# jihun1998/AO

Measured on AMD Instinct MI355X. Metric: points/sec fwd+bwd PTv2m2 S3DIS, higher is better.
Workload: dtype fp32

## Files before the change

### ao_amd/csrc/gemm.hip

```cpp
#include <algorithm>

#include "common.h"

namespace gemm {

constexpr int BM = 64;
constexpr int THREADS = 256;
template <int KC>
__device__ __forceinline__ int lds_slot(int row, int k4) {
    return row * (KC + 8) + 4 * (k4 ^ (row & (KC == 32 ? 1 : 3)));
}

typedef float v4f __attribute__((ext_vector_type(4)));

struct GemmMulti {
    const float *X[3], *W[3], *bias[3];
    float *Y[3];
    int count;
    int sum;
    const float *xsc, *xsh;
    float *stats[3];
    const float *bnx, *bnm, *bnr, *bng, *bnb;
    int bnrelu;
    float *brec;
};

template <int CTRL>
__device__ __forceinline__ float dpp_mov(float v) {
    return __int_as_float(__builtin_amdgcn_update_dpp(0, __float_as_int(v), CTRL, 0xF, 0xF, true));
}
__device__ __forceinline__ float row16_sum(float v) {
    v += dpp_mov<0xB1>(v);
    v += dpp_mov<0x4E>(v);
    v += dpp_mov<0x141>(v);
    v += dpp_mov<0x140>(v);
    return v;
}

template <int BN>
// ... 11 lines not shown
        float4 v = make_float4(acc[t][0], acc[t][1], acc[t][2], acc[t][3]);
        {
            const float4 bb = ptv2_ld_or_zero((const float4 *)(bias + col), bias && col < n);
            v.x += bb.x; v.y += bb.y; v.z += bb.z; v.w += bb.w;
        }
        val[t] = v;
        if (row < m && col < n) {
            float4 *dst = (float4 *)(Y + row * n + col);
            if (accumulate) {
                const float4 o = *dst;
                v.x += o.x; v.y += o.y; v.z += o.z; v.w += o.w;
            }
            *dst = v;
        }
    }
    if (multi.count && multi.brec) {
        float *sS = sX;
        const bool rv = row < m;
        const int cl = (lane >> 4) * 4;
        __syncthreads();
#pragma unroll
        for (int t = 0; t < NT; ++t) {
            const int col = n0 + t * 16 + cl;
            float4 d = make_float4(0.f, 0.f, 0.f, 0.f), e = d;
            if (rv && col < n) {
                const float4 xv = *(const float4 *)(multi.bnx + row * n + col);
                const float4 mm = *(const float4 *)(multi.bnm + col), rs = *(const float4 *)(multi.bnr + col);
                float4 h;
                h.x = (xv.x - mm.x) * rs.x; h.y = (xv.y - mm.y) * rs.y; h.z = (xv.z - mm.z) * rs.z; h.w = (xv.w - mm.w) * rs.w;
                d = val[t];
                if (multi.bnrelu) {
                    const float4 gg = *(const float4 *)(multi.bng + col), bb = *(const float4 *)(multi.bnb + col);
                    if (__builtin_fmaf(h.x, gg.x, bb.x) <= 0.f) d.x = 0.f;
                    if (__builtin_fmaf(h.y, gg.y, bb.y) <= 0.f) d.y = 0.f;
                    if (__builtin_fmaf(h.z, gg.z, bb.z) <= 0.f) d.z = 0.f;
                    if (__builtin_fmaf(h.w, gg.w, bb.w) <= 0.f) d.w = 0.f;
                }
                e = make_float4(d.x * h.x, d.y * h.y, d.z * h.z, d.w * h.w);
            }
            const float ax = row16_sum(d.x), ay = row16_sum(d.y), az = row16_sum(d.z), aw = row16_sum(d.w);
            const float bx = row16_sum(e.x), by = row16_sum(e.y), bz = row16_sum(e.z), bw = row16_sum(e.w);
            if ((lane & 15) == 0) {
                *(float4 *)(sS + (wid * 2 + 0) * BN + t * 16 + cl) = make_float4(ax, ay, az, aw);
                *(float4 *)(sS + (wid * 2 + 1) * BN + t * 16 + cl) = make_float4(bx, by, bz, bw);
            }
        }
        __syncthreads();
        for (int e = tid; e < 2 * BN; e += THREADS) {
            const int which = e / BN, cc = e - which * BN;
            if (n0 + cc < n) {
                float a = sS[which * BN + cc];
#pragma unroll
                for (int w = 1; w < 4; ++w) a += sS[(w * 2 + which) * BN + cc];
                multi.brec[(size_t)rb * 2 * n + (size_t)which * n + n0 + cc] = a;
            }
        }
    }
    float *stats = multi.count ? multi.stats[indep ? z : 0] : nullptr;
    if (stats) {
        float *sS = sX;
        const bool rv = row < m;
        const int cnt = (int)((m - row0) < BM ? (m - row0) : BM);
        const int cl = (lane >> 4) * 4;
        __syncthreads();
#pragma unroll
        for (int t = 0; t < NT; ++t) {
            const float sx = row16_sum(rv ? val[t].x : 0.f), sy = row16_sum(rv ? val[t].y : 0.f);
            const float sz = row16_sum(rv ? val[t].z : 0.f), sw = row16_sum(rv ? val[t].w : 0.f);
            if ((lane & 15) == 0) *(float4 *)(sS + wid * BN + t * 16 + cl) = make_float4(sx, sy, sz, sw);
// ... 29 lines not shown
                if (col < n) {
                    float4 a = *(const float4 *)(sS + t * 16 + cl);
#pragma unroll
                    for (int w = 1; w < 4; ++w) {
                        const float4 o = *(const float4 *)(sS + w * BN + t * 16 + cl);
                        a.x += o.x; a.y += o.y; a.z += o.z; a.w += o.w;
                    }
                    *(float4 *)(stats + (size_t)rb * 2 * n + n + col) = a;
                }
            }
        }
    }
}

template <int BN, bool W_KMAJOR, int KC, bool BF16>
__global__ __launch_bounds__(THREADS) void rows_gemm_kernel(int m, int n, int k, const float *__restrict__ X0,
                                                            const float *__restrict__ W0,
                                                            const float *__restrict__ bias0, float *__restrict__ Y0,
                                                            int accumulate, int ncb, GemmMulti multi) {
    constexpr int PITCH = KC + 8;
    __shared__ __attribute__((aligned(16))) float sX[BM * PITCH];
    __shared__ __attribute__((aligned(16))) float sW[BN * PITCH];
    constexpr int NT = BN / 16;
    constexpr int KQ = KC / 4;
    constexpr int XLOADS = BM * KQ / THREADS;
    constexpr int WQ = BN * KQ;
    constexpr int WLOADS = (WQ + THREADS - 1) / THREADS;
    constexpr int RUN = KC / 16;
    const int tid = threadIdx.x, lane = tid & 63, wid = tid >> 6;
    const int rb = blockIdx.x / ncb, cb = blockIdx.x - rb * ncb;
    const long long row0 = (long long)rb * BM;
    const int n0 = cb * BN;
    const int z = blockIdx.y;
    const bool indep = multi.count && !multi.sum;
    const float *bias = indep ? multi.bias[z] : bias0;
    float *Y = multi.count ? multi.Y[indep ? z : 0] : Y0;
    const int npair = (multi.count && multi.sum) ? multi.count : 1;
    const float *X = multi.count ? multi.X[indep ? z : 0] : X0;
    const float *W = multi.count ? multi.W[indep ? z : 0] : W0;

    float4 rx[XLOADS], rw[WLOADS];
    auto fetch = [&](int k0) {
#pragma unroll
        for (int j = 0; j < XLOADS; ++j) {
            const int q = tid + j * THREADS, r = q / KQ, kq = (q % KQ) * 4;
            const long long row = row0 + r;
            rx[j] = ptv2_ld_or_zero((const float4 *)(X + row * k + k0 + kq), row < m && k0 + kq < k);
            if (multi.xsc && k0 + kq < k) {
                const float4 s4 = *(const float4 *)(multi.xsc + k0 + kq), h4 = *(const float4 *)(multi.xsh + k0 + kq);
                rx[j].x = fmaxf(__builtin_fmaf(rx[j].x, s4.x, h4.x), 0.f);
                rx[j].y = fmaxf(__builtin_fmaf(rx[j].y, s4.y, h4.y), 0.f);
                rx[j].z = fmaxf(__builtin_fmaf(rx[j].z, s4.z, h4.z), 0.f);
                rx[j].w = fmaxf(__builtin_fmaf(rx[j].w, s4.w, h4.w), 0.f);
            }
        }
#pragma unroll
        for (int j = 0; j < WLOADS; ++j) {
            const int q = tid + j * THREADS;
            {
                if (!W_KMAJOR) {
                    const int r = q / KQ, kq = (q % KQ) * 4;
                    rw[j] = ptv2_ld_or_zero((const float4 *)(W + (long long)(n0 + r) * k + k0 + kq), q < WQ && n0 + r < n && k0 + kq < k);
                } else {
                    const int kk = q % KC, cq = (q / KC) * 4;
// ... 71 lines not shown
                        acc[t] = __builtin_amdgcn_mfma_f32_16x16x4f32(w4.x, xr[j].x, acc[t], 0, 0, 0);
                        acc[t] = __builtin_amdgcn_mfma_f32_16x16x4f32(w4.y, xr[j].y, acc[t], 0, 0, 0);
                        acc[t] = __builtin_amdgcn_mfma_f32_16x16x4f32(w4.z, xr[j].z, acc[t], 0, 0, 0);
                        acc[t] = __builtin_amdgcn_mfma_f32_16x16x4f32(w4.w, xr[j].w, acc[t], 0, 0, 0);
                    }
                }
            }
            if (more) {
                __syncthreads();
                stash();
                __syncthreads();
            }
        }
    }
    gemm_epilogue<BN>(acc, row0, rb, n0, z, indep, m, n, bias, Y, accumulate, multi, sX);
}

template <int BN, bool W_KMAJOR, int K, bool BF16>
__global__ __launch_bounds__(THREADS) void rows_gemm_direct_kernel(int m, int n, const float *__restrict__ X0,
                                                                   const float *__restrict__ W0, const float *__restrict__ bias0,
                                                                   float *__restrict__ Y0, int accumulate, int ncb, GemmMulti multi) {
    constexpr int NT = BN / 16, QF = K / 16, LDW = K + 8, KQ = K / 4;
    extern __shared__ float4 gd_lds4[];
    float *sW = (float *)gd_lds4;
    float *sSc = sW + (size_t)BN * LDW;
    const int tid = threadIdx.x, lane = tid & 63, wid = tid >> 6, l15 = lane & 15, q = lane >> 4;
    const int rb = blockIdx.x / ncb, cb = blockIdx.x - rb * ncb;
    const long long row0 = (long long)rb * BM;
    const int n0 = cb * BN;
    const int z = blockIdx.y;
    const bool indep = multi.count && !multi.sum;
    const float *bias = indep ? multi.bias[z] : bias0;
    float *Y = multi.count ? multi.Y[indep ? z : 0] : Y0;
    const int npair = (multi.count && multi.sum) ? multi.count : 1;
    const float *X = multi.count ? multi.X[indep ? z : 0] : X0;
    const float *W = multi.count ? multi.W[indep ? z : 0] : W0;
    const long long row = row0 + wid * 16 + l15;
    const bool rv = row < m;

    v4f acc[NT];
#pragma unroll
    for (int t = 0; t < NT; ++t) acc[t] = (v4f){0.f, 0.f, 0.f, 0.f};
    if (multi.xsc)
        for (int e = tid; e < K; e += THREADS) { sSc[e] = multi.xsc[e]; sSc[K + e] = multi.xsh[e]; }
    for (int pair = 0; pair < npair; ++pair) {
        if (pair > 0) {
            X = multi.X[pair];
            W = multi.W[pair];
            __syncthreads();
        }
        float4 x[QF];
        const float *xr = rv ? X + row * K + 4 * q : ptv2_zero_pad;
#pragma unroll
        for (int j = 0; j < QF; ++j) x[j] = *(const float4 *)(xr + 16 * j);
        if (!W_KMAJOR) {
            constexpr int WL = (BN * KQ + THREADS - 1) / THREADS;
#pragma unroll
            for (int b0 = 0; b0 < WL; b0 += 8) {
                float4 w4[8];
// ... 27 lines not shown
                }
#pragma unroll
                for (int i = 0; i < 8; ++i) {
                    if (b0 + i < WL) {
                        const int e = tid + (b0 + i) * THREADS;
                        const int kk = e % K, cq = (e / K) * 4;
                        if (e < (BN / 4) * K) {
                            sW[(size_t)(cq + 0) * LDW + kk] = w4[i].x; sW[(size_t)(cq + 1) * LDW + kk] = w4[i].y;
                            sW[(size_t)(cq + 2) * LDW + kk] = w4[i].z; sW[(size_t)(cq + 3) * LDW + kk] = w4[i].w;
                        }
                    }
                }
            }
        }
        __syncthreads();
        if (multi.xsc) {
#pragma unroll
            for (int j = 0; j < QF; ++j) {
                const float4 s4 = *(const float4 *)(sSc + 16 * j + 4 * q), h4 = *(const float4 *)(sSc + K + 16 * j + 4 * q);
                x[j].x = fmaxf(__builtin_fmaf(x[j].x, s4.x, h4.x), 0.f); x[j].y = fmaxf(__builtin_fmaf(x[j].y, s4.y, h4.y), 0.f);
                x[j].z = fmaxf(__builtin_fmaf(x[j].z, s4.z, h4.z), 0.f); x[j].w = fmaxf(__builtin_fmaf(x[j].w, s4.w, h4.w), 0.f);
            }
        }
        const float *pw = sW + (size_t)l15 * LDW + 4 * q;
        if constexpr (BF16) {
#pragma unroll
            for (int j = 0; j < QF; j += 2) {
                const float4 x1 = j + 1 < QF ? x[j + 1] : make_float4(0.f, 0.f, 0.f, 0.f);
                const ptv2_bf16x8 xb = ptv2_pack_bf16(x[j], x1);
#pragma unroll
                for (int t = 0; t < NT; ++t) {
// ... 26 lines not shown
                                                                   int ncb, GemmMulti multi) {
    constexpr int NT = BN / 16, QF = K / 16, JW = (QF + 3) / 4;
    __shared__ __attribute__((aligned(16))) float sRed[4][NT][64 * 4];
    const int tid = threadIdx.x, lane = tid & 63, wid = tid >> 6, l15 = lane & 15, q = lane >> 4;
    const int rb = blockIdx.x / ncb, cb = blockIdx.x - rb * ncb;
    const long long row0 = (long long)rb * 16;
    const int n0 = cb * BN;
    const int z = blockIdx.y;
    const bool indep = multi.count && !multi.sum;
    const float *bias = indep ? multi.bias[z] : bias0;
    float *Y = multi.count ? multi.Y[indep ? z : 0] : Y0;
    const int npair = (multi.count && multi.sum) ? multi.count : 1;
    const long long row = row0 + l15;
    const bool rv = row < m;
    const int j0 = wid * JW;
    v4f acc[NT];
#pragma unroll
    for (int t = 0; t < NT; ++t) acc[t] = (v4f){0.f, 0.f, 0.f, 0.f};
    for (int pair = 0; pair < npair; ++pair) {
        const float *X = multi.count ? multi.X[indep ? z : pair] : X0;
        const float *W = multi.count ? multi.W[indep ? z : pair] : W0;
        float4 x[JW], w[JW][NT], s4[JW], h4[JW];
        const float *xr = rv ? X + row * K + 4 * q : ptv2_zero_pad;
#pragma unroll
        for (int jj = 0; jj < JW; ++jj) {
            const int j = j0 + jj;
            const bool jok = j < QF;
            x[jj] = *(const float4 *)((jok && rv) ? xr + 16 * j : ptv2_zero_pad);
            if (multi.xsc) {
                s4[jj] = *(const float4 *)(jok ? multi.xsc + 16 * j + 4 * q : ptv2_zero_pad);
                h4[jj] = *(const float4 *)(jok ? multi.xsh + 16 * j + 4 * q : ptv2_zero_pad);
            }
#pragma unroll
            for (int t = 0; t < NT; ++t) {
                const int col = n0 + 16 * t + l15;
                const bool ok = jok && col < n;
                if (!W_KMAJOR) {
                    w[jj][t] = *(const float4 *)(ok ? W + (long long)col * K + 16 * j + 4 * q : ptv2_zero_pad);
                } else {
                    const float *wp = ok ? W + (long long)(16 * j + 4 * q) * n + col : ptv2_zero_pad;
                    const long long st = ok ? n : 0;
                    w[jj][t] = make_float4(wp[0], wp[st], wp[2 * st], wp[3 * st]);
                }
            }
        }
#pragma unroll
        for (int jj = 0; jj < JW; ++jj) {
            if (multi.xsc) {
                x[jj].x = fmaxf(__builtin_fmaf(x[jj].x, s4[jj].x, h4[jj].x), 0.f); x[jj].y = fmaxf(__builtin_fmaf(x[jj].y, s4[jj].y, h4[jj].y), 0.f);
                x[jj].z = fmaxf(__builtin_fmaf(x[jj].z, s4[jj].z, h4[jj].z), 0.f); x[jj].w = fmaxf(__builtin_fmaf(x[jj].w, s4[jj].w, h4[jj].w), 0.f);
                if (!rv) x[jj] = make_float4(0.f, 0.f, 0.f, 0.f);
            }
#pragma unroll
            for (int t = 0; t < NT; ++t) {
                acc[t] = __builtin_amdgcn_mfma_f32_16x16x4f32(w[jj][t].x, x[jj].x, acc[t], 0, 0, 0);
                acc[t] = __builtin_amdgcn_mfma_f32_16x16x4f32(w[jj][t].y, x[jj].y, acc[t], 0, 0, 0);
                acc[t] = __builtin_amdgcn_mfma_f32_16x16x4f32(w[jj][t].z, x[jj].z, acc[t], 0, 0, 0);
                acc[t] = __builtin_amdgcn_mfma_f32_16x16x4f32(w[jj][t].w, x[jj].w, acc[t], 0, 0, 0);
            }
        }
    }
#pragma unroll
    for (int t = 0; t < NT; ++t) *(float4 *)(&sRed[wid][t][4 * lane]) = make_float4(acc[t][0], acc[t][1], acc[t][2], acc[t][3]);
    __syncthreads();
    float *stats = multi.count ? multi.stats[indep ? z : 0] : nullptr;
    const int cnt = (int)((m - row0) < 16 ? (m - row0) : 16);
    const float inv = 1.0f / (float)cnt;
#pragma unroll
    for (int t = 0; t < NT; ++t) {
        if ((t & 3) != wid) continue;
        const float4 a0 = *(const float4 *)(&sRed[0][t][4 * lane]), a1 = *(const float4 *)(&sRed[1][t][4 * lane]);
        const float4 a2 = *(const float4 *)(&sRed[2][t][4 * lane]), a3 = *(const float4 *)(&sRed[3][t][4 * lane]);
        const int col = n0 + 16 * t + 4 * q;
        const bool cok = col < n;
        float4 v = make_float4(((a0.x + a1.x) + a2.x) + a3.x, ((a0.y + a1.y) + a2.y) + a3.y, ((a0.z + a1.z) + a2.z) + a3.z,
                               ((a0.w + a1.w) + a2.w) + a3.w);
        {
            const float4 bb = ptv2_ld_or_zero((const float4 *)(bias + col), bias && cok);
            v.x += bb.x; v.y += bb.y; v.z += bb.z; v.w += bb.w;
        }
        const float4 val = v;
        if (rv && cok) {
            float4 *dst = (float4 *)(Y + row * n + col);
            if (accumulate) {
                const float4 o = *dst;
                v.x += o.x; v.y += o.y; v.z += o.z; v.w += o.w;
            }
            *dst = v;
        }
        if (multi.count && multi.brec) {
            float4 d = make_float4(0.f, 0.f, 0.f, 0.f), e = d;
            if (rv && cok) {
                const float4 xv = *(const float4 *)(multi.bnx + row * n + col);
                const float4 mm = *(const float4 *)(multi.bnm + col), rs = *(const float4 *)(multi.bnr + col);
                float4 h;
                h.x = (xv.x - mm.x) * rs.x; h.y = (xv.y - mm.y) * rs.y; h.z = (xv.z - mm.z) * rs.z; h.w = (xv.w - mm.w) * rs.w;
                d = val;
                if (multi.bnrelu) {
                    const float4 gg = *(const float4 *)(multi.bng + col), bb = *(const float4 *)(multi.bnb + col);
                    if (__builtin_fmaf(h.x, gg.x, bb.x) <= 0.f) d.x = 0.f;
                    if (__builtin_fmaf(h.y, gg.y, bb.y) <= 0.f) d.y = 0.f;
                    if (__builtin_fmaf(h.z, gg.z, bb.z) <= 0.f) d.z = 0.f;
                    if (__builtin_fmaf(h.w, gg.w, bb.w) <= 0.f) d.w = 0.f;
                }
                e = make_float4(d.x * h.x, d.y * h.y, d.z * h.z, d.w * h.w);
            }
            const float ax = row16_sum(d.x), ay = row16_sum(d.y), az = row16_sum(d.z), aw = row16_sum(d.w);
            const float bx = row16_sum(e.x), by = row16_sum(e.y), bz = row16_sum(e.z), bw = row16_sum(e.w);
            if (l15 == 0 && cok) {
                *(float4 *)(multi.brec + (size_t)rb * 2 * n + col) = make_float4(ax, ay, az, aw);
                *(float4 *)(multi.brec + (size_t)rb * 2 * n + n + col) = make_float4(bx, by, bz, bw);
            }
        }
        if (stats) {
            const float sx = row16_sum(rv ? val.x : 0.f), sy = row16_sum(rv ? val.y : 0.f);
            const float sz = row16_sum(rv ? val.z : 0.f), sw = row16_sum(rv ? val.w : 0.f);
            const float dx = rv ? val.x - sx * inv : 0.f, dy = rv ? val.y - sy * inv : 0.f;
            const float dz = rv ? val.z - sz * inv : 0.f, dw = rv ? val.w - sw * inv : 0.f;
            const float qx = row16_sum(dx * dx), qy = row16_sum(dy * dy), qz = row16_sum(dz * dz), qw = row16_sum(dw * dw);
            if (l15 == 0 && cok) {
                *(float4 *)(stats + (size_t)rb * 2 * n + col) = make_float4(sx, sy, sz, sw);
                *(float4 *)(stats + (size_t)rb * 2 * n + n + col) = make_float4(qx, qy, qz, qw);
            }
        }
    }
}
// ... 95 lines not shown
#define GO(BN, KM, KC) launch_one<BN, KM, KC>(grid, st, m, n, k, X, W, bias, Y, accumulate, ncb, gm)
    if (bn == 16) {
        if (kmajor) { if (wide_k) GO(16, true, 64); else GO(16, true, 32); }
        else { if (wide_k) GO(16, false, 64); else GO(16, false, 32); }
    } else if (bn == 32) {
        if (kmajor) { if (wide_k) GO(32, true, 64); else GO(32, true, 32); }
        else { if (wide_k) GO(32, false, 64); else GO(32, false, 32); }
    } else if (bn == 48) {
        if (kmajor) { if (wide_k) GO(48, true, 64); else GO(48, true, 32); }
        else { if (wide_k) GO(48, false, 64); else GO(48, false, 32); }
    } else {
        if (kmajor) { if (wide_k) GO(64, true, 64); else GO(64, true, 32); }
        else { if (wide_k) GO(64, false, 64); else GO(64, false, 32); }
    }
#undef GO
}

extern "C" int rows_gemm_hip_launcher(int m, int n, int k, const float *X, const float *W, int w_kmajor,
                                      const float *bias, float *Y, int accumulate, void *stream) {
    using namespace gemm;
    if (m < 0 || n < 4 || k < 4 || n % 4 != 0 || k % 4 != 0 || !X || !W || !Y) return PTV2_ERR_ARG;
    if (m == 0) return PTV2_OK;
    hipStream_t st = (hipStream_t)stream;
    const bool n48 = n % 48 == 0;
    const int bn = column_block(m, n);
    const int ncb = (n + bn - 1) / bn;
    const long long nrb = ((long long)m + BM - 1) / BM;
    if (nrb * ncb > 2147483647LL) return PTV2_ERR_ARG;
    const dim3 grid((unsigned)(nrb * ncb));
    {
// ... 10 lines not shown
                                            const float *const *W, int w_kmajor, const float *const *bias, float *const *Y,
                                            int accumulate, const float *xsc, const float *xsh, float *const *stats,
                                            void *stream) {
    using namespace gemm;
    if (m < 0 || n < 4 || k < 4 || n % 4 != 0 || k % 4 != 0 || count < 1 || count > 3 || !X || !W || !Y) return PTV2_ERR_ARG;
    if (m == 0) return PTV2_OK;
    GemmMulti gm{};
    gm.count = count;
    gm.sum = sum ? 1 : 0;
    for (int i = 0; i < count; ++i) {
        if (!X[i] || !W[i] || (!Y[i] && (i == 0 || !sum))) return PTV2_ERR_ARG;
        gm.X[i] = X[i]; gm.W[i] = W[i]; gm.bias[i] = bias ? bias[i] : nullptr; gm.Y[i] = Y[i];
        gm.stats[i] = stats ? stats[i] : nullptr;
    }
    if ((xsc == nullptr) != (xsh == nullptr)) return PTV2_ERR_ARG;
    gm.xsc = xsc;
    gm.xsh = xsh;
    hipStream_t st = (hipStream_t)stream;
    const bool n48 = n % 48 == 0;
    const int bn = column_block(m, n, sum ? 1 : count);
    const int ncb = (n + bn - 1) / bn;
    const long long nrb = ((long long)m + BM - 1) / BM;
    if (nrb * ncb > 2147483647LL) return PTV2_ERR_ARG;
    const dim3 grid((unsigned)(nrb * ncb), sum ? 1 : count);
    const float *b0 = sum ? gm.bias[0] : nullptr;
    {
        PtvScopedTimer t(KID_ROWS_GEMM + (n48 ? 0 : 4) + (w_kmajor ? 2 : 0) + (k >= 192 ? 1 : 0), st,
                         4.0 * count * ((double)m * (n + k) + (double)n * k));
        bool records = false;
        for (int i = 0; i < count; ++i) records = records || gm.stats[i] != nullptr;
        if (!try_ksplit(m, n, k, w_kmajor != 0, sum ? 1 : count, st, gm.X[0], gm.W[0], b0, gm.Y[0], accumulate, gm, records))
            launch_gemm(bn, w_kmajor != 0, k >= 192, grid, st, m, n, k, gm.X[0], gm.W[0], b0, gm.Y[0], accumulate, ncb, gm);
// ... 12 lines not shown
extern "C" int rows_gemm_bnbwd_hip_launcher(int m, int n, int k, int count, const float *const *X, const float *const *W,
                                            int w_kmajor, float *Y, const float *bn_x, const float *bn_mean, const float *bn_rstd,
                                            const float *bn_gamma, const float *bn_beta, int relu, float *records, void *stream) {
    using namespace gemm;
    if (m < 0 || n < 4 || k < 4 || n % 4 != 0 || k % 4 != 0 || count < 1 || count > 3 || !X || !W || !Y) return PTV2_ERR_ARG;
    if (!bn_x || !bn_mean || !bn_rstd || !records || (relu && (!bn_gamma || !bn_beta))) return PTV2_ERR_ARG;
    if (m == 0) return PTV2_OK;
    GemmMulti gm{};
    gm.count = count;
    gm.sum = 1;
    for (int i = 0; i < count; ++i) {
        if (!X[i] || !W[i]) return PTV2_ERR_ARG;
        gm.X[i] = X[i]; gm.W[i] = W[i];
    }
    gm.Y[0] = Y;
    gm.bnx = bn_x; gm.bnm = bn_mean; gm.bnr = bn_rstd; gm.bng = bn_gamma; gm.bnb = bn_beta; gm.bnrelu = relu; gm.brec = records;
    hipStream_t st = (hipStream_t)stream;
    const bool n48 = n % 48 == 0;
    const int bn = column_block(m, n);
    const int ncb = (n + bn - 1) / bn;
    const long long nrb = ((long long)m + BM - 1) / BM;
    if (nrb * ncb > 2147483647LL) return PTV2_ERR_ARG;
    const dim3 grid((unsigned)(nrb * ncb), 1);
    {
        PtvScopedTimer t(KID_ROWS_GEMM + (n48 ? 0 : 4) + (w_kmajor ? 2 : 0) + (k >= 192 ? 1 : 0), st,
                         4.0 * ((double)m * (2 * n + count * k) + (double)count * n * k));
        if (!try_ksplit(m, n, k, w_kmajor != 0, 1, st, gm.X[0], gm.W[0], nullptr, Y, 0, gm, true))
            launch_gemm(bn, w_kmajor != 0, k >= 192, grid, st, m, n, k, gm.X[0], gm.W[0], nullptr, Y, 0, ncb, gm);
    }
    PTV2_CHECK_LAUNCH();
    return PTV2_OK;
// ... 2 lines not shown
```

### ao_amd/csrc/internal.h

```cpp
#pragma once

struct GvaPlan;
namespace gva {
struct FoldWFwdArgs; struct FoldWBwdArgs; struct PtvDrop;
struct AttnIn; struct AttnFwdOut; struct AttnBwdIn; struct AttnBwdOut;
struct LogitsIn; struct LogitsOut; struct LogitsBwdIn; struct LogitsBwdOut;
}
namespace dense { struct WgradJob; struct BnTileSet; }

void ptv2_profile_scope(int which, int end, int ring_entry, int ring_size);
int rows_gemm_record_rows(int m, int n, int k);
void ptv2_gemm_allow_rb16(int on);
size_t bn_tiles_floats_rb(int n, int c, int rb);
int bn_tiles_finalize_rb(int n, int c, const dense::BnTileSet &S, float eps, float momentum, void *stream);
int bn_tiles_finalize_pair(int n, int c, const dense::BnTileSet (&S)[2], float eps, float momentum, void *stream);
int bn_tiles_apply_residual(int n, int c, const dense::BnTileSet &S, float eps, float momentum, const float *x,
                            const float *residual, const float *rowscale, float *y, void *stream);
int bn_tiles_apply_relu(int n, int c, const dense::BnTileSet &S, float eps, float momentum, const float *x, float *y, void *stream);
int skinny_linear_forward_pair(int n, int cin, int cout, const float *const *x, const float *W, const float *const *xsc,
                               const float *const *xsh, float *const *y, void *stream);
void ptv2_skinny_bn_arm(int n, int c, const float *const *x, const float *const *gy, const float *const *mean,
                        const float *const *rstd, const float *const *gamma, const float *const *beta, int relu, void *workspace,
                        size_t workspace_bytes);
void ptv2_skinny_bn_disarm(void);
struct PtvSkinnyBnScope {
    PtvSkinnyBnScope() = default;
    ~PtvSkinnyBnScope() { ptv2_skinny_bn_disarm(); }
// ... 63 lines not shown
```

### ao_amd/csrc/skinny.hip

```cpp
#include "dense_common.h"

namespace dense {

__global__ __launch_bounds__(TPB) void skinny_fwd_kernel(long long n, int cin, int cout, const float *x, const float *__restrict__ W,
                                                         const float *xsc, const float *xsh, float *y, const float *x2,
                                                         const float *xsc2, const float *xsh2, float *y2) {
    extern __shared__ float4 lds4[];
    if (blockIdx.y) { x = x2; xsc = xsc2; xsh = xsh2; y = y2; }
    float *sW = (float *)lds4;
    const int ldw = cin + 4, cq = cin >> 2;
    float *sSc = sW + (size_t)cout * ldw, *sSh = sSc + cin;
    for (int e = threadIdx.x; e < cout * cq; e += TPB) {
        const int r = e / cq, q = e - r * cq;
        *(float4 *)(sW + (size_t)r * ldw + 4 * q) = *(const float4 *)(W + (size_t)r * cin + 4 * q);
    }
    if (xsc)
        for (int e = threadIdx.x; e < cin; e += TPB) { sSc[e] = xsc[e]; sSh[e] = xsh[e]; }
    __syncthreads();
    const long long total = n * cout;
    for (long long e = (long long)blockIdx.x * TPB + threadIdx.x; e < total; e += (long long)gridDim.x * TPB) {
        const long long row = e / cout;
        const int o = (int)(e - row * cout);
        const float4 *xr = (const float4 *)(x + row * cin), *wr = (const float4 *)(sW + (size_t)o * ldw);
        float acc = 0.f;
// ... 134 lines not shown
    const size_t lds = sizeof(float) * ((size_t)cout * (cin + 4) + 2 * (size_t)cin);
    if (lds > 160 * 1024) return PTV2_ERR_ARG;
    if (lds > 32 * 1024)
        (void)hipFuncSetAttribute((const void *)skinny_fwd_kernel, hipFuncAttributeMaxDynamicSharedMemorySize, (int)lds);
    const long long total = (long long)n * cout;
    const int nblk = (int)std::min<long long>((total + TPB - 1) / TPB, 256 * 8);
    {
        PtvScopedTimer t(KID_SKINNY_FWD, (hipStream_t)stream, 4.0 * n * (cin + cout));
        hipLaunchKernelGGL(skinny_fwd_kernel, dim3(nblk), dim3(TPB), lds, (hipStream_t)stream, (long long)n, cin, cout, x, W, xsc,
                           xsh, y, (const float *)nullptr, (const float *)nullptr, (const float *)nullptr, (float *)nullptr);
    }
    PTV2_CHECK_LAUNCH();
    return PTV2_OK;
}

int skinny_linear_forward_pair(int n, int cin, int cout, const float *const *x, const float *W, const float *const *xsc,
                               const float *const *xsh, float *const *y, void *stream) {
    if (n < 0 || cin < 4 || cin % 4 != 0 || cout < 1 || cout > 64) return PTV2_ERR_ARG;
    if ((xsc[0] == nullptr) != (xsc[1] == nullptr)) return PTV2_ERR_ARG;
    if (n == 0) return PTV2_OK;
    const size_t lds = sizeof(float) * ((size_t)cout * (cin + 4) + 2 * (size_t)cin);
    if (lds > 160 * 1024) return PTV2_ERR_ARG;
    if (lds > 32 * 1024)
        (void)hipFuncSetAttribute((const void *)skinny_fwd_kernel, hipFuncAttributeMaxDynamicSharedMemorySize, (int)lds);
    const long long total = (long long)n * cout;
    const int nblk = (int)std::min<long long>((total + TPB - 1) / TPB, 256 * 8);
    {
        PtvScopedTimer t(KID_SKINNY_FWD, (hipStream_t)stream, 8.0 * n * (cin + cout));
        hipLaunchKernelGGL(skinny_fwd_kernel, dim3(nblk, 2), dim3(TPB), lds, (hipStream_t)stream, (long long)n, cin, cout, x[0], W,
                           xsc[0], xsh[0], y[0], x[1], xsc[1], xsh[1], y[1]);
    }
    PTV2_CHECK_LAUNCH();
    return PTV2_OK;
}

extern "C" int skinny_linear_forward_hip_launcher(int n, int cin, int cout, const float *x, const float *W, float *y,
                                                 void *stream) {
    return skinny_linear_forward_xf_hip_launcher(n, cin, cout, x, W, nullptr, nullptr, y, stream);
}

extern "C" int skinny_linear_backward_hip_launcher(int n, int cin, int cout, const float *gy, const float *W, float *gx,
                                                  void *stream) {
    if (n < 0 || cin < 4 || cin % 4 != 0 || cout < 1) return PTV2_ERR_ARG;
    if (n == 0) return PTV2_OK;
    const long long total = (long long)n * (cin >> 2);
    const int nblk = apply_grid(total);
    {
        PtvScopedTimer t(KID_SKINNY_BWD, (hipStream_t)stream, 4.0 * n * (cin + cout));
// ... 34 lines not shown
    K = SkinnyBnArm{};
    static const bool off = ptv2_env_is("AO_AMD_SKINNY_BN", '0');
    if (off || n < 1 || c < 4 || c % 4 != 0 || (c >> 2) > TPB || !workspace || workspace_bytes < dense_workspace_bytes(n, 2 * c, c)) return;
    K.armed = true;
    K.n = n; K.c = c; K.nblk = bn_grid(n, c); K.relu = relu;
    constexpr int cap = 256;
    if (n <= 16384) {
        const int rl = std::max(1, TPB / (c >> 2));
        K.nblk = (int)std::max<long long>(1, std::min<long long>(((long long)n + rl * 2 - 1) / (rl * 2), cap));
    }
    for (int i = 0; i < 2; ++i) { K.x[i] = x[i]; K.gy[i] = gy[i]; K.mean[i] = mean[i]; K.rstd[i] = rstd[i]; K.gamma[i] = gamma[i]; K.beta[i] = beta[i]; }
    K.part = (float *)workspace;
}
void ptv2_skinny_bn_disarm(void) { t_skinny_bn.armed = false; }

int skinny_backward_pair_bn_reduce(int n, int cin, int cout, const float *const *gy, const float *W, float *const *gx, void *stream) {
    SkinnyBnArm &K = t_skinny_bn;
    const bool fuse = K.armed && K.n == n && K.c == cin && K.gy[0] == gx[0] && K.gy[1] == gx[1] && n > 0;
    K.armed = false;
    if (!fuse) return skinny_linear_backward_pair(n, cin, cout, gy, W, gx, stream);
    hipStream_t st = (hipStream_t)stream;
    {
        PtvScopedTimer t(KID_SKINNY_BWD, st, 8.0 * n * (cin + cout) + 8.0 * n * cin);
        const gva::PtvRiders Rs = gva::ptv2_rider_take();
        const SkinnyBn A{gy[0], gx[0], K.x[0], K.mean[0], K.rstd[0], K.gamma[0], K.beta[0]};
        const SkinnyBn B{gy[1], gx[1], K.x[1], K.mean[1], K.rstd[1], K.gamma[1], K.beta[1]};
        hipLaunchKernelGGL(skinny_bn_bwd_reduce_kernel, dim3(K.nblk + gva::rider_blocks(Rs), 2), dim3(TPB), sizeof(float4) * 2 * TPB, st,
                           n, cin, cout, A, B, W, K.relu, K.part, K.nblk, Rs);
    }
    K.done = true;
    PTV2_CHECK_LAUNCH();
    return PTV2_OK;
}

int ptv2_skinny_bn_take_records(int n, int c, const float *part, const float *const *gy) {
    SkinnyBnArm &K = t_skinny_bn;
    const bool reduced = K.done && K.part == part && K.n == n && K.c == c && K.gy[0] == gy[0] && K.gy[1] == gy[1];
    K.done = false;
    return reduced ? K.nblk : 0;
}
```

Baseline: 12.81 million.

## Route skinny pair linear fwd/bwd through MFMA rows-GEMM kernels with BN fusion

Adds a selector that sends the paired skinny linear forward and the BN-fused backward to the existing rows-GEMM MFMA kernels (direct, k-split or LDS forms chosen by input width). GemmMulti gains per-pair pointers for input scale/shift, BN tensors and record buffers so both pairs run in one launch via blockIdx.y. A new riders kernel variant appends rider blocks to the backward GEMM grid. The aim is to replace the scalar skinny kernels with matrix-core GEMMs, at the cost of more code paths and a different BN record layout with its own block count.

```diff
diff --git a/ao_amd/csrc/gemm.hip b/ao_amd/csrc/gemm.hip
--- a/ao_amd/csrc/gemm.hip
+++ b/ao_amd/csrc/gemm.hip
@@ -1,6 +1,7 @@
 #include <algorithm>
 
 #include "common.h"
+#include "gva_common.h"
 
 namespace gemm {
 
@@ -18,11 +19,12 @@
     float *Y[3];
     int count;
     int sum;
-    const float *xsc, *xsh;
+    const float *xsc[3], *xsh[3];
     float *stats[3];
-    const float *bnx, *bnm, *bnr, *bng, *bnb;
+    const float *bnx[3], *bnm[3], *bnr[3], *bng[3], *bnb[3];
     int bnrelu;
-    float *brec;
+    float *brec[3];
+    int brec_stride;
 };
 
 template <int CTRL>
@@ -64,7 +66,11 @@
             *dst = v;
         }
     }
-    if (multi.count && multi.brec) {
+    const int zb = indep ? z : 0;
+    float *brec = multi.count ? multi.brec[zb] : nullptr;
+    if (brec) {
+        const float *bnx = multi.bnx[zb], *bnm = multi.bnm[zb], *bnr = multi.bnr[zb], *bng = multi.bng[zb], *bnb = multi.bnb[zb];
+        const size_t rstride = multi.brec_stride ? (size_t)multi.brec_stride : 2 * (size_t)n;
         float *sS = sX;
         const bool rv = row < m;
         const int cl = (lane >> 4) * 4;
@@ -74,13 +80,13 @@
             const int col = n0 + t * 16 + cl;
             float4 d = make_float4(0.f, 0.f, 0.f, 0.f), e = d;
             if (rv && col < n) {
-                const float4 xv = *(const float4 *)(multi.bnx + row * n + col);
-                const float4 mm = *(const float4 *)(multi.bnm + col), rs = *(const float4 *)(multi.bnr + col);
+                const float4 xv = *(const float4 *)(bnx + row * n + col);
+                const float4 mm = *(const float4 *)(bnm + col), rs = *(const float4 *)(bnr + col);
                 float4 h;
                 h.x = (xv.x - mm.x) * rs.x; h.y = (xv.y - mm.y) * rs.y; h.z = (xv.z - mm.z) * rs.z; h.w = (xv.w - mm.w) * rs.w;
                 d = val[t];
                 if (multi.bnrelu) {
-                    const float4 gg = *(const float4 *)(multi.bng + col), bb = *(const float4 *)(multi.bnb + col);
+                    const float4 gg = *(const float4 *)(bng + col), bb = *(const float4 *)(bnb + col);
                     if (__builtin_fmaf(h.x, gg.x, bb.x) <= 0.f) d.x = 0.f;
                     if (__builtin_fmaf(h.y, gg.y, bb.y) <= 0.f) d.y = 0.f;
                     if (__builtin_fmaf(h.z, gg.z, bb.z) <= 0.f) d.z = 0.f;
@@ -102,7 +108,7 @@
                 float a = sS[which * BN + cc];
 #pragma unroll
                 for (int w = 1; w < 4; ++w) a += sS[(w * 2 + which) * BN + cc];
-                multi.brec[(size_t)rb * 2 * n + (size_t)which * n + n0 + cc] = a;
+                brec[(size_t)rb * rstride + (size_t)which * n + n0 + cc] = a;
             }
         }
     }
@@ -162,10 +168,9 @@
 }
 
 template <int BN, bool W_KMAJOR, int KC, bool BF16>
-__global__ __launch_bounds__(THREADS) void rows_gemm_kernel(int m, int n, int k, const float *__restrict__ X0,
-                                                            const float *__restrict__ W0,
-                                                            const float *__restrict__ bias0, float *__restrict__ Y0,
-                                                            int accumulate, int ncb, GemmMulti multi) {
+__device__ __forceinline__ void rows_gemm_tile(const int bx, int m, int n, int k, const float *__restrict__ X0,
+                                               const float *__restrict__ W0, const float *__restrict__ bias0,
+                                               float *__restrict__ Y0, int accumulate, int ncb, const GemmMulti &multi) {
     constexpr int PITCH = KC + 8;
     __shared__ __attribute__((aligned(16))) float sX[BM * PITCH];
     __shared__ __attribute__((aligned(16))) float sW[BN * PITCH];
@@ -176,7 +181,7 @@
     constexpr int WLOADS = (WQ + THREADS - 1) / THREADS;
     constexpr int RUN = KC / 16;
     const int tid = threadIdx.x, lane = tid & 63, wid = tid >> 6;
-    const int rb = blockIdx.x / ncb, cb = blockIdx.x - rb * ncb;
+    const int rb = bx / ncb, cb = bx - rb * ncb;
     const long long row0 = (long long)rb * BM;
     const int n0 = cb * BN;
     const int z = blockIdx.y;
@@ -186,6 +191,7 @@
     const int npair = (multi.count && multi.sum) ? multi.count : 1;
     const float *X = multi.count ? multi.X[indep ? z : 0] : X0;
     const float *W = multi.count ? multi.W[indep ? z : 0] : W0;
+    const float *xsc = multi.xsc[indep ? z : 0], *xsh = multi.xsh[indep ? z : 0];
 
     float4 rx[XLOADS], rw[WLOADS];
     auto fetch = [&](int k0) {
@@ -194,8 +200,8 @@
             const int q = tid + j * THREADS, r = q / KQ, kq = (q % KQ) * 4;
             const long long row = row0 + r;
             rx[j] = ptv2_ld_or_zero((const float4 *)(X + row * k + k0 + kq), row < m && k0 + kq < k);
-            if (multi.xsc && k0 + kq < k) {
-                const float4 s4 = *(const float4 *)(multi.xsc + k0 + kq), h4 = *(const float4 *)(multi.xsh + k0 + kq);
+            if (xsc && k0 + kq < k) {
+                const float4 s4 = *(const float4 *)(xsc + k0 + kq), h4 = *(const float4 *)(xsh + k0 + kq);
                 rx[j].x = fmaxf(__builtin_fmaf(rx[j].x, s4.x, h4.x), 0.f);
                 rx[j].y = fmaxf(__builtin_fmaf(rx[j].y, s4.y, h4.y), 0.f);
                 rx[j].z = fmaxf(__builtin_fmaf(rx[j].z, s4.z, h4.z), 0.f);
@@ -297,6 +303,24 @@
         }
     }
     gemm_epilogue<BN>(acc, row0, rb, n0, z, indep, m, n, bias, Y, accumulate, multi, sX);
+}
+
+template <int BN, bool W_KMAJOR, int KC, bool BF16>
+__global__ __launch_bounds__(THREADS) void rows_gemm_kernel(int m, int n, int k, const float *__restrict__ X0,
+                                                            const float *__restrict__ W0,
+                                                            const float *__restrict__ bias0, float *__restrict__ Y0,
+                                                            int accumulate, int ncb, GemmMulti multi) {
+    rows_gemm_tile<BN, W_KMAJOR, KC, BF16>((int)blockIdx.x, m, n, k, X0, W0, bias0, Y0, accumulate, ncb, multi);
+}
+
+template <int BN>
+__global__ __launch_bounds__(THREADS) void rows_gemm_riders_kernel(int m, int n, int k, int ncb, GemmMulti multi, int main_blocks,
+                                                                   gva::PtvRiders Rs) {
+    if ((int)blockIdx.x >= main_blocks) {
+        if (blockIdx.y == 0) gva::rider_run(Rs, (int)blockIdx.x - main_blocks);
+        return;
+    }
+    rows_gemm_tile<BN, true, 32, false>((int)blockIdx.x, m, n, k, nullptr, nullptr, nullptr, nullptr, 0, ncb, multi);
 }
 
 template <int BN, bool W_KMAJOR, int K, bool BF16>
@@ -324,8 +348,9 @@
     v4f acc[NT];
 #pragma unroll
     for (int t = 0; t < NT; ++t) acc[t] = (v4f){0.f, 0.f, 0.f, 0.f};
-    if (multi.xsc)
-        for (int e = tid; e < K; e += THREADS) { sSc[e] = multi.xsc[e]; sSc[K + e] = multi.xsh[e]; }
+    const float *xsc = multi.xsc[indep ? z : 0], *xsh = multi.xsh[indep ? z : 0];
+    if (xsc)
+        for (int e = tid; e < K; e += THREADS) { sSc[e] = xsc[e]; sSc[K + e] = xsh[e]; }
     for (int pair = 0; pair < npair; ++pair) {
         if (pair > 0) {
             X = multi.X[pair];
@@ -383,7 +408,7 @@
             }
         }
         __syncthreads();
-        if (multi.xsc) {
+        if (xsc) {
 #pragma unroll
             for (int j = 0; j < QF; ++j) {
                 const float4 s4 = *(const float4 *)(sSc + 16 * j + 4 * q), h4 = *(const float4 *)(sSc + K + 16 * j + 4 * q);
@@ -440,6 +465,7 @@
     const long long row = row0 + l15;
     const bool rv = row < m;
     const int j0 = wid * JW;
+    const float *xsc = multi.xsc[indep ? z : 0], *xsh = multi.xsh[indep ? z : 0];
     v4f acc[NT];
 #pragma unroll
     for (int t = 0; t < NT; ++t) acc[t] = (v4f){0.f, 0.f, 0.f, 0.f};
@@ -453,9 +479,9 @@
             const int j = j0 + jj;
             const bool jok = j < QF;
             x[jj] = *(const float4 *)((jok && rv) ? xr + 16 * j : ptv2_zero_pad);
-            if (multi.xsc) {
-                s4[jj] = *(const float4 *)(jok ? multi.xsc + 16 * j + 4 * q : ptv2_zero_pad);
-                h4[jj] = *(const float4 *)(jok ? multi.xsh + 16 * j + 4 * q : ptv2_zero_pad);
+            if (xsc) {
+                s4[jj] = *(const float4 *)(jok ? xsc + 16 * j + 4 * q : ptv2_zero_pad);
+                h4[jj] = *(const float4 *)(jok ? xsh + 16 * j + 4 * q : ptv2_zero_pad);
             }
 #pragma unroll
             for (int t = 0; t < NT; ++t) {
@@ -472,7 +498,7 @@
         }
 #pragma unroll
         for (int jj = 0; jj < JW; ++jj) {
-            if (multi.xsc) {
+            if (xsc) {
                 x[jj].x = fmaxf(__builtin_fmaf(x[jj].x, s4[jj].x, h4[jj].x), 0.f); x[jj].y = fmaxf(__builtin_fmaf(x[jj].y, s4[jj].y, h4[jj].y), 0.f);
                 x[jj].z = fmaxf(__builtin_fmaf(x[jj].z, s4[jj].z, h4[jj].z), 0.f); x[jj].w = fmaxf(__builtin_fmaf(x[jj].w, s4[jj].w, h4[jj].w), 0.f);
                 if (!rv) x[jj] = make_float4(0.f, 0.f, 0.f, 0.f);
@@ -490,6 +516,10 @@
     for (int t = 0; t < NT; ++t) *(float4 *)(&sRed[wid][t][4 * lane]) = make_float4(acc[t][0], acc[t][1], acc[t][2], acc[t][3]);
     __syncthreads();
     float *stats = multi.count ? multi.stats[indep ? z : 0] : nullptr;
+    const int zb = indep ? z : 0;
+    float *brec = multi.count ? multi.brec[zb] : nullptr;
+    const float *bnx = multi.bnx[zb], *bnm = multi.bnm[zb], *bnr = multi.bnr[zb], *bng = multi.bng[zb], *bnb = multi.bnb[zb];
+    const size_t rstride = multi.brec_stride ? (size_t)multi.brec_stride : 2 * (size_t)n;
     const int cnt = (int)((m - row0) < 16 ? (m - row0) : 16);
     const float inv = 1.0f / (float)cnt;
 #pragma unroll
@@ -514,16 +544,16 @@
             }
             *dst = v;
         }
-        if (multi.count && multi.brec) {
+        if (brec) {
             float4 d = make_float4(0.f, 0.f, 0.f, 0.f), e = d;
             if (rv && cok) {
-                const float4 xv = *(const float4 *)(multi.bnx + row * n + col);
-                const float4 mm = *(const float4 *)(multi.bnm + col), rs = *(const float4 *)(multi.bnr + col);
+                const float4 xv = *(const float4 *)(bnx + row * n + col);
+                const float4 mm = *(const float4 *)(bnm + col), rs = *(const float4 *)(bnr + col);
                 float4 h;
                 h.x = (xv.x - mm.x) * rs.x; h.y = (xv.y - mm.y) * rs.y; h.z = (xv.z - mm.z) * rs.z; h.w = (xv.w - mm.w) * rs.w;
                 d = val;
                 if (multi.bnrelu) {
-                    const float4 gg = *(const float4 *)(multi.bng + col), bb = *(const float4 *)(multi.bnb + col);
+                    const float4 gg = *(const float4 *)(bng + col), bb = *(const float4 *)(bnb + col);
                     if (__builtin_fmaf(h.x, gg.x, bb.x) <= 0.f) d.x = 0.f;
                     if (__builtin_fmaf(h.y, gg.y, bb.y) <= 0.f) d.y = 0.f;
                     if (__builtin_fmaf(h.z, gg.z, bb.z) <= 0.f) d.z = 0.f;
@@ -534,8 +564,8 @@
             const float ax = row16_sum(d.x), ay = row16_sum(d.y), az = row16_sum(d.z), aw = row16_sum(d.w);
             const float bx = row16_sum(e.x), by = row16_sum(e.y), bz = row16_sum(e.z), bw = row16_sum(e.w);
             if (l15 == 0 && cok) {
-                *(float4 *)(multi.brec + (size_t)rb * 2 * n + col) = make_float4(ax, ay, az, aw);
-                *(float4 *)(multi.brec + (size_t)rb * 2 * n + n + col) = make_float4(bx, by, bz, bw);
+                *(float4 *)(brec + (size_t)rb * rstride + col) = make_float4(ax, ay, az, aw);
+                *(float4 *)(brec + (size_t)rb * rstride + n + col) = make_float4(bx, by, bz, bw);
             }
         }
         if (stats) {
@@ -661,6 +691,71 @@
         else { if (wide_k) GO(64, false, 64); else GO(64, false, 32); }
     }
 #undef GO
+}
+
+int rows_gemm_pair_forward(int form, int m, int n, int k, const float *const *X, const float *W, const float *const *xsc,
+                           const float *const *xsh, float *const *Y, void *stream) {
+    using namespace gemm;
+    const int kind = form / 100, bn = form % 100;
+    if (m < 1 || n < 4 || n % 4 != 0 || (k != 96 && k != 192 && k != 384) || !X || !W || !xsc || !xsh || !Y) return PTV2_ERR_ARG;
+    if (bn != 16 && bn != 32 && bn != 48 && bn != 64) return PTV2_ERR_ARG;
+    if (kind == GEMM_FORM_DIRECT && bn != 16 && bn != 48) return PTV2_ERR_ARG;
+    GemmMulti gm{};
+    gm.count = 2;
+    for (int i = 0; i < 2; ++i) {
+        if (!X[i] || !Y[i] || !xsc[i] || !xsh[i]) return PTV2_ERR_ARG;
+        gm.X[i] = X[i]; gm.W[i] = W; gm.Y[i] = Y[i]; gm.xsc[i] = xsc[i]; gm.xsh[i] = xsh[i];
+    }
+    const PtvMatmulScope fp32(0);
+    hipStream_t st = (hipStream_t)stream;
+    const int ncb = (n + bn - 1) / bn, rows = kind == GEMM_FORM_KSPLIT ? 16 : BM;
+    const dim3 grid((unsigned)(((m + rows - 1) / rows) * ncb), 2);
+#define PF(CALL) do { if (bn == 16) { CALL(16); } else if (bn == 32) { CALL(32); } else if (bn == 48) { CALL(48); } else { CALL(64); } } while (0)
+#define PF_LDS(BN) do { if (k >= 192) launch_one<BN, false, 64>(grid, st, m, n, k, X[0], W, nullptr, Y[0], 0, ncb, gm); \
+                        else launch_one<BN, false, 32>(grid, st, m, n, k, X[0], W, nullptr, Y[0], 0, ncb, gm); } while (0)
+#define PF_DIRECT(BN) do { if (k == 96) launch_direct<BN, false, 96>(grid, st, m, n, X[0], W, nullptr, Y[0], 0, ncb, gm); \
+                           else if (k == 192) launch_direct<BN, false, 192>(grid, st, m, n, X[0], W, nullptr, Y[0], 0, ncb, gm); \
+                           else launch_direct<BN, false, 384>(grid, st, m, n, X[0], W, nullptr, Y[0], 0, ncb, gm); } while (0)
+#define PF_KSPLIT(BN) launch_ksplit_k<BN, false>(k, grid, st, m, n, X[0], W, nullptr, Y[0], 0, ncb, gm)
+    switch (kind) {
+        case GEMM_FORM_LDS: PF(PF_LDS); break;
+        case GEMM_FORM_DIRECT: if (bn == 16) PF_DIRECT(16); else PF_DIRECT(48); break;
+        case GEMM_FORM_KSPLIT: PF(PF_KSPLIT); break;
+        default: return PTV2_ERR_ARG;
+    }
+#undef PF_KSPLIT
+#undef PF_DIRECT
+#undef PF_LDS
+    PTV2_CHECK_LAUNCH();
+    return PTV2_OK;
+}
+
+int rows_gemm_pair_bnbwd(int form, int m, int n, int k, const float *const *X, const float *W, float *const *Y, const float *const *bn_x,
+                         const float *const *bn_mean, const float *const *bn_rstd, const float *const *bn_gamma,
+                         const float *const *bn_beta, int relu, float *records, const gva::PtvRiders &Rs, void *stream) {
+    using namespace gemm;
+    const int kind = form / 100, bn = form % 100;
+    if (m < 1 || n < 4 || n % 4 != 0 || k < 4 || k % 4 != 0 || k > 64 || !X || !W || !Y || !records) return PTV2_ERR_ARG;
+    if (kind != GEMM_FORM_LDS || (bn != 16 && bn != 32 && bn != 48 && bn != 64)) return PTV2_ERR_ARG;
+    GemmMulti gm{};
+    gm.count = 2;
+    gm.bnrelu = relu;
+    gm.brec_stride = 4 * n;
+    for (int i = 0; i < 2; ++i) {
+        if (!X[i] || !Y[i] || !bn_x[i] || !bn_mean[i] || !bn_rstd[i] || (relu && (!bn_gamma[i] || !bn_beta[i]))) return PTV2_ERR_ARG;
+        gm.X[i] = X[i]; gm.W[i] = W; gm.Y[i] = Y[i];
+        gm.bnx[i] = bn_x[i]; gm.bnm[i] = bn_mean[i]; gm.bnr[i] = bn_rstd[i]; gm.bng[i] = bn_gamma[i]; gm.bnb[i] = bn_beta[i];
+        gm.brec[i] = records + (size_t)i * 2 * n;
+    }
+    const int ncb = (n + bn - 1) / bn;
+    const int main_blocks = ((m + BM - 1) / BM) * ncb;
+    const dim3 grid((unsigned)(main_blocks + gva::rider_blocks(Rs)), 2);
+#define PB(BN) hipLaunchKernelGGL(rows_gemm_riders_kernel<BN>, grid, dim3(THREADS), 0, (hipStream_t)stream, m, n, k, ncb, gm, main_blocks, Rs)
+    PF(PB);
+#undef PB
+#undef PF
+    PTV2_CHECK_LAUNCH();
+    return PTV2_OK;
 }
 
 extern "C" int rows_gemm_hip_launcher(int m, int n, int k, const float *X, const float *W, int w_kmajor,
@@ -701,8 +796,7 @@
         gm.stats[i] = stats ? stats[i] : nullptr;
     }
     if ((xsc == nullptr) != (xsh == nullptr)) return PTV2_ERR_ARG;
-    gm.xsc = xsc;
-    gm.xsh = xsh;
+    for (int i = 0; i < 3; ++i) { gm.xsc[i] = xsc; gm.xsh[i] = xsh; }
     hipStream_t st = (hipStream_t)stream;
     const bool n48 = n % 48 == 0;
     const int bn = column_block(m, n, sum ? 1 : count);
@@ -745,7 +839,8 @@
         gm.X[i] = X[i]; gm.W[i] = W[i];
     }
     gm.Y[0] = Y;
-    gm.bnx = bn_x; gm.bnm = bn_mean; gm.bnr = bn_rstd; gm.bng = bn_gamma; gm.bnb = bn_beta; gm.bnrelu = relu; gm.brec = records;
+    gm.bnx[0] = bn_x; gm.bnm[0] = bn_mean; gm.bnr[0] = bn_rstd; gm.bng[0] = bn_gamma; gm.bnb[0] = bn_beta; gm.bnrelu = relu;
+    gm.brec[0] = records;
     hipStream_t st = (hipStream_t)stream;
     const bool n48 = n % 48 == 0;
     const int bn = column_block(m, n);
diff --git a/ao_amd/csrc/internal.h b/ao_amd/csrc/internal.h
--- a/ao_amd/csrc/internal.h
+++ b/ao_amd/csrc/internal.h
@@ -2,7 +2,7 @@
 
 struct GvaPlan;
 namespace gva {
-struct FoldWFwdArgs; struct FoldWBwdArgs; struct PtvDrop;
+struct FoldWFwdArgs; struct FoldWBwdArgs; struct PtvDrop; struct PtvRiders;
 struct AttnIn; struct AttnFwdOut; struct AttnBwdIn; struct AttnBwdOut;
 struct LogitsIn; struct LogitsOut; struct LogitsBwdIn; struct LogitsBwdOut;
 }
@@ -11,6 +11,12 @@
 void ptv2_profile_scope(int which, int end, int ring_entry, int ring_size);
 int rows_gemm_record_rows(int m, int n, int k);
 void ptv2_gemm_allow_rb16(int on);
+enum { GEMM_FORM_LDS = 1, GEMM_FORM_DIRECT = 2, GEMM_FORM_KSPLIT = 3 };
+int rows_gemm_pair_forward(int form, int m, int n, int k, const float *const *X, const float *W, const float *const *xsc,
+                           const float *const *xsh, float *const *Y, void *stream);
+int rows_gemm_pair_bnbwd(int form, int m, int n, int k, const float *const *X, const float *W, float *const *Y, const float *const *bn_x,
+                         const float *const *bn_mean, const float *const *bn_rstd, const float *const *bn_gamma,
+                         const float *const *bn_beta, int relu, float *records, const gva::PtvRiders &Rs, void *stream);
 size_t bn_tiles_floats_rb(int n, int c, int rb);
 int bn_tiles_finalize_rb(int n, int c, const dense::BnTileSet &S, float eps, float momentum, void *stream);
 int bn_tiles_finalize_pair(int n, int c, const dense::BnTileSet (&S)[2], float eps, float momentum, void *stream);
diff --git a/ao_amd/csrc/skinny.hip b/ao_amd/csrc/skinny.hip
--- a/ao_amd/csrc/skinny.hip
+++ b/ao_amd/csrc/skinny.hip
@@ -172,11 +172,30 @@
     return PTV2_OK;
 }
 
-int skinny_linear_forward_pair(int n, int cin, int cout, const float *const *x, const float *W, const float *const *xsc,
-                               const float *const *xsh, float *const *y, void *stream) {
+struct SkinnyMfmaPick { int fwd, bwd; };
+static SkinnyMfmaPick skinny_mfma_pick(int n, int cin, int cout) {
+    static const bool off = ptv2_env_is("AO_AMD_SKINNY_MFMA", '0'), fwd_only = ptv2_env_is("AO_AMD_SKINNY_MFMA", 'f');
+    SkinnyMfmaPick P{0, 0};
+    if (off || n < 1 || cout % 4 != 0 || cout > 64 || (cin != 96 && cin != 192 && cin != 384)) return P;
+    const bool rec_room = ((long long)n + 63) / 64 <= MAX_BLK;
+    switch (cin) {
+        case 96: P.fwd = 100 * GEMM_FORM_DIRECT + 16; P.bwd = 0; break;
+        case 192: P.fwd = 100 * GEMM_FORM_KSPLIT + 32; P.bwd = 100 * GEMM_FORM_LDS + 32; break;
+        default: P.fwd = 0; P.bwd = 100 * GEMM_FORM_LDS + 16; break;
+    }
+    if (fwd_only || !rec_room) P.bwd = 0;
+    return P;
+}
+
+static int skinny_forward_pair_form(int form, int n, int cin, int cout, const float *const *x, const float *W, const float *const *xsc,
+                                    const float *const *xsh, float *const *y, void *stream) {
     if (n < 0 || cin < 4 || cin % 4 != 0 || cout < 1 || cout > 64) return PTV2_ERR_ARG;
     if ((xsc[0] == nullptr) != (xsc[1] == nullptr)) return PTV2_ERR_ARG;
     if (n == 0) return PTV2_OK;
+    if (form && xsc[0] && xsh[0] && xsh[1]) {
+        PtvScopedTimer t(KID_SKINNY_FWD, (hipStream_t)stream, 8.0 * n * (cin + cout));
+        return rows_gemm_pair_forward(form, n, cout, cin, x, W, xsc, xsh, y, stream);
+    }
     const size_t lds = sizeof(float) * ((size_t)cout * (cin + 4) + 2 * (size_t)cin);
     if (lds > 160 * 1024) return PTV2_ERR_ARG;
     if (lds > 32 * 1024)
@@ -190,6 +209,11 @@
     }
     PTV2_CHECK_LAUNCH();
     return PTV2_OK;
+}
+
+int skinny_linear_forward_pair(int n, int cin, int cout, const float *const *x, const float *W, const float *const *xsc,
+                               const float *const *xsh, float *const *y, void *stream) {
+    return skinny_forward_pair_form(skinny_mfma_pick(n, cin, cout).fwd, n, cin, cout, x, W, xsc, xsh, y, stream);
 }
 
 extern "C" int skinny_linear_forward_hip_launcher(int n, int cin, int cout, const float *x, const float *W, float *y,
@@ -254,12 +278,21 @@
 }
 void ptv2_skinny_bn_disarm(void) { t_skinny_bn.armed = false; }
 
-int skinny_backward_pair_bn_reduce(int n, int cin, int cout, const float *const *gy, const float *W, float *const *gx, void *stream) {
+static int skinny_backward_pair_form(int form, int n, int cin, int cout, const float *const *gy, const float *W, float *const *gx,
+                                     void *stream) {
     SkinnyBnArm &K = t_skinny_bn;
     const bool fuse = K.armed && K.n == n && K.c == cin && K.gy[0] == gx[0] && K.gy[1] == gx[1] && n > 0;
     K.armed = false;
     if (!fuse) return skinny_linear_backward_pair(n, cin, cout, gy, W, gx, stream);
     hipStream_t st = (hipStream_t)stream;
+    if (form) {
+        PtvScopedTimer t(KID_SKINNY_BWD, st, 8.0 * n * (cin + cout) + 8.0 * n * cin);
+        K.nblk = (n + 63) / 64;
+        const gva::PtvRiders Rs = gva::ptv2_rider_take();
+        RUN(rows_gemm_pair_bnbwd(form, n, cin, cout, gy, W, gx, K.x, K.mean, K.rstd, K.gamma, K.beta, K.relu, K.part, Rs, stream));
+        K.done = true;
+        return PTV2_OK;
+    }
     {
         PtvScopedTimer t(KID_SKINNY_BWD, st, 8.0 * n * (cin + cout) + 8.0 * n * cin);
         const gva::PtvRiders Rs = gva::ptv2_rider_take();
@@ -273,6 +306,34 @@
     return PTV2_OK;
 }
 
+int skinny_backward_pair_bn_reduce(int n, int cin, int cout, const float *const *gy, const float *W, float *const *gx, void *stream) {
+    return skinny_backward_pair_form(skinny_mfma_pick(n, cin, cout).bwd, n, cin, cout, gy, W, gx, stream);
+}
+
+extern "C" int skinny_pair_form(int backward, int n, int cin, int cout) {
+    const SkinnyMfmaPick P = skinny_mfma_pick(n, cin, cout);
+    return backward ? P.bwd : P.fwd;
+}
+extern "C" int skinny_pair_forward_form_hip_launcher(int form, int n, int cin, int cout, const float *const *x, const float *W,
+                                                     const float *const *xsc, const float *const *xsh, float *const *y, void *stream) {
+    if (!x || !W || !xsc || !xsh || !y) return PTV2_ERR_ARG;
+    return skinny_forward_pair_form(form < 0 ? skinny_mfma_pick(n, cin, cout).fwd : form, n, cin, cout, x, W, xsc, xsh, y, stream);
+}
+extern "C" int skinny_pair_backward_form_hip_launcher(int form, int n, int cin, int cout, const float *const *sg, const float *W,
+                                                      float *const *gy, const float *const *bn_x, const float *const *bn_mean,
+                                                      const float *const *bn_rstd, const float *const *bn_gamma,
+                                                      const float *const *bn_beta, int relu, void *records, size_t records_bytes,
+                                                      int *nrec, void *stream) {
+    if (!sg || !W || !gy || !bn_x || !bn_mean || !bn_rstd || !bn_gamma || !bn_beta || !records || !nrec) return PTV2_ERR_ARG;
+    const float *gyc[2] = {gy[0], gy[1]};
+    ptv2_skinny_bn_arm(n, cin, bn_x, gyc, bn_mean, bn_rstd, bn_gamma, bn_beta, relu, records, records_bytes);
+    const PtvSkinnyBnScope scope;
+    if (!t_skinny_bn.armed) return PTV2_ERR_WORKSPACE;
+    RUN(skinny_backward_pair_form(form < 0 ? skinny_mfma_pick(n, cin, cout).bwd : form, n, cin, cout, sg, W, gy, stream));
+    *nrec = ptv2_skinny_bn_take_records(n, cin, (const float *)records, gyc);
+    return PTV2_OK;
+}
+
 int ptv2_skinny_bn_take_records(int n, int c, const float *part, const float *const *gy) {
     SkinnyBnArm &K = t_skinny_bn;
     const bool reduced = K.done && K.part == part && K.n == n && K.c == c && K.gy[0] == gy[0] && K.gy[1] == gy[1];
```

Result: no change. 12.92 million (median of 6 runs) (+0.9%).
